# DavidSevic/gpu-nbody-simulation

Measured on AMD Instinct MI355X. Metric: body-steps/sec, higher is better.
Workload: dtype f32

## Files before the change

gpu-nbody-simulation_amd/csrc/bh_engine.hip:

```cpp
#include "../../include/bhgpu.h"

#include <hip/hip_runtime.h>

#include <algorithm>
#include <cmath>
#include <cstdio>
#include <cstdlib>
#include <cstring>
#include <string>
#include <type_traits>
#include <vector>

#include "bh_tree.hpp"
#include "bh_walk_exact.hpp"
#include "bh_walk_f64.hpp"
#include "bh_diag.hpp"
#include "bh_direct.hpp"
#include "bh_field.hpp"
#include "bh_init.hpp"
#include "bh_let.hpp"
#include "bh_migrate.hpp"
#include "bh_walk_fast.h"

using namespace bh;
// ... 18 lines not shown
};

}

struct bh_ctx {
    bh_config cfg{};
    int Dm = 0;
    enum class Mode { Exact, F64, Mixed, F32 };
    Mode mode = Mode::Exact;
    bool tree64() const { return mode == Mode::Exact || mode == Mode::F64; }
    bool state64() const { return mode != Mode::F32; }
    bool compat = true;
    bool exact_thresholds = false;
    int device = 0;
    hipStream_t stream = nullptr;
    bool own_stream = false;
    int64_t n = 0;
    bool uploaded = false, tree_valid = false;
    int64_t internal_cap = 0, node_cap = 0;
    int64_t bfs_max = 12288;
    int exact_bpw = 0;
    int walk_split = 0;
    bool walk_asm = true;
    int sort_bucket = 1;
    bool last_sort_bucket = false, last_sort_packed = false;
    int64_t samples_n = -1;
    uint64_t *splitters = nullptr;
    uint16_t *sort_dig = nullptr;
    int build_items = 0;
    bool hilbert = false;
    int partial_count = 0;
    double *bslots = nullptr;
    bool slots_valid = false;
    bool slots_dirty = true;

    void *pos = nullptr, *vel = nullptr, *mass = nullptr, *force = nullptr;
    void *pos2 = nullptr, *vel2 = nullptr, *mass2 = nullptr, *force2 = nullptr;
    uint32_t *orig = nullptr, *orig2 = nullptr;
    bool orig_identity = true;
    int reorder_every = 16;
    int64_t builds = 0;
    float2 *spos = nullptr;
    float4 *sstate = nullptr;
    float *smass = nullptr;
    uint64_t *keys[2] = {nullptr, nullptr};
    uint32_t *vals[2] = {nullptr, nullptr};
// ... 477 lines not shown
        }, c->compat);
        return BH_OK;
    });
}

int launch_walk_f32(bh_ctx *c, const WalkRange &w, const WalkChoice &k)
{
    WalkFastArgs a{};
    a.quads = c->qf; a.aux = c->aux; a.partial = w.partial; a.spos = c->spos; a.smass = c->smass; a.perm = c->perm;
    a.pos = (float2 *)c->pos; a.vel = (float2 *)c->vel;
    a.state64 = c->state64() ? 1 : 0;
    a.sstate = c->sstate;
    a.acc_out = (float2 *)c->force; a.ctr = c->ctr;
    a.lo = w.lo; a.hi = w.hi; a.G = (float)c->cfg.G; a.dt = (float)c->cfg.dt;
    a.integrate = w.integrate ? 1 : 0; a.to_sorted = w.to_sorted ? 1 : 0;
    a.n_trees = c->let_mode ? c->world : 0; a.self_rank = c->let_mode ? c->rank : -1;
    a.part = w.part; a.acc_part = c->acc_part;
    a.forest_base = c->forest_base; a.let_cap = c->let_cap;
    c->exp.walk_args(a);
    a.group_cost = (w.lo == 0 && w.hi == c->n) ? c->group_cost : nullptr;
    a.bucket_consts = c->walk_consts;
    a.slots = w.slots;
    a.body_counts = w.stats ? c->body_counts : nullptr;
    const bool lds = (c->cfg.flags & BH_FLAG_LDS_STACK) != 0;
    a.pair_limit = std::max(0, 116 - 3 * c->Dm);
    int split = (c->cfg.flags & BH_FLAG_WALK_NO_SPLIT) || c->cfg.n_threads > 0 ? 1 : c->walk_split;
    if (split <= 0) {
        const int64_t groups = (w.hi - w.lo + kWave - 1) / kWave;
        split = groups <= (c->let_mode ? 512 : 768) ? 8 : groups <= 3072 ? 4 : 1;
    }
    if (3 * c->Dm + 2 > kWave) split = 1;
    const int per_record = walk_fast_split_effective(a, lds, split) ? kWave : kBlock;
    if (w.partial) c->partial_count = (int)blocks_for(w.hi - w.lo, per_record);
    return each_pass(c, w, per_record, [&](int64_t plo, int64_t phi, unsigned) -> int {
        a.lo = plo; a.hi = phi; a.partial = w.partial ? w.partial + 4 * ((plo - w.lo) / per_record) : nullptr;
        BH_HIP(c, launch_walk_fast(a, lds, w.stats, split, k.use_asm, c->stream));
        return BH_OK;
    });
}

int enqueue_walk(bh_ctx *c, bool integrate, bool to_sorted, int part = 0)
{
    WalkRange w{};
    owned_range(c, &w.lo, &w.hi);
    if (w.hi <= w.lo) return BH_OK;
    w.integrate = integrate; w.to_sorted = to_sorted; w.part = part;
// ... 79 lines not shown
    if (cfg->max_depth < 1 || cfg->max_depth > 32)
        return fail(nullptr, BH_ERR_ARG, "bh_create: max_depth must be 1..32");
    if (!(cfg->theta > 0.0)) return fail(nullptr, BH_ERR_ARG, "bh_create: theta must be > 0");
    if (cfg->precision != BH_PRECISION_F64_EXACT && cfg->precision != BH_PRECISION_F32 &&
        cfg->precision != BH_PRECISION_MIXED && cfg->precision != BH_PRECISION_F64)
        return fail(nullptr, BH_ERR_ARG, "bh_create: unknown precision");
    int ndev = 0;
    if (hipGetDeviceCount(&ndev) != hipSuccess || ndev <= 0)
        return fail(nullptr, BH_ERR_NO_DEVICE, "bh_create: no HIP device (libbhgpu has no CPU fallback)");
    if (cfg->device < 0 || cfg->device >= ndev)
        return fail(nullptr, BH_ERR_ARG, "bh_create: device ordinal out of range");

    bh_ctx *c = new bh_ctx();
    c->cfg = *cfg;
    c->Dm = cfg->max_depth - 1;
    c->mode = cfg->precision == BH_PRECISION_F64_EXACT ? Mode::Exact
            : cfg->precision == BH_PRECISION_F64       ? Mode::F64
            : cfg->precision == BH_PRECISION_MIXED     ? Mode::Mixed : Mode::F32;
    c->compat = cfg->reference_compat != 0;
    c->device = cfg->device;
    if (const char *e = std::getenv("BH_WALK_SPLIT")) c->walk_split = std::atoi(e);
    if (const char *e = std::getenv("BH_EXACT_BPW")) { const int b = std::atoi(e); c->exact_bpw = (b >= 1 && b <= kWave && (b & (b - 1)) == 0) ? b : 0; }
    if (const char *e = std::getenv("BH_WALK_ASM")) c->walk_asm = std::atoi(e) != 0;
    if (const char *e = std::getenv("BH_EXACT_BFS_MAX")) c->bfs_max = std::max(0, std::atoi(e));
    c->exact_thresholds = c->mode == Mode::Exact && c->walk_asm && !(cfg->flags & BH_FLAG_WALK_PORTABLE);
    if (const char *e = std::getenv("BH_SORT_PACK")) c->sort_pack = std::atoi(e) != 0;
    if (const char *e = std::getenv("BH_SORT_BUCKET")) c->sort_bucket = std::atoi(e);
    if (const char *e = std::getenv("BH_BUILD_ITEMS")) c->build_items = std::atoi(e);
    if (const char *e = std::getenv("BH_REORDER_EVERY")) c->reorder_every = std::max(0, std::atoi(e));
    c->hilbert = !c->tree64();
    if (const char *e = std::getenv("BH_HILBERT")) c->hilbert = !c->tree64() && std::atoi(e) != 0;
    auto bail = [&](int rc) { g_create_error = c->err; bh_destroy(c); return rc; };

    if (hipSetDevice(c->device) != hipSuccess) { c->err = "hipSetDevice failed"; return bail(BH_ERR_DEVICE); }
    if (hipStreamCreateWithFlags(&c->stream, hipStreamNonBlocking) != hipSuccess) {
        c->err = "hipStreamCreate failed"; return bail(BH_ERR_DEVICE);
    }
    c->own_stream = true;

    const int64_t cap = std::max<int64_t>(cfg->capacity, 1);
    c->node_cap = cfg->node_capacity > 0 ? cfg->node_capacity : 8 * cap + 1024;
    if (c->Dm < 15) {
        int64_t full = 0, wdt = 1;
        for (int l = 0; l <= c->Dm; ++l) { full += wdt; wdt *= 4; }
        c->node_cap = std::min(c->node_cap, std::max<int64_t>(full, 1));
    }
    c->internal_cap = (c->node_cap - 1) / 4;

    const size_t rs = c->state64() ? sizeof(double) : sizeof(float);
    int rc = 0;
    auto A = [&](auto **pp, size_t count) { if (!rc) rc = dev_alloc(c, pp, count); };
    { char *t; A(&t, cap * 2 * rs); c->pos = t; }
    { char *t; A(&t, cap * 2 * rs); c->vel = t; }
    { char *t; A(&t, cap * rs); c->mass = t; }
    { char *t; A(&t, cap * 2 * (c->tree64() ? sizeof(double) : sizeof(float))); c->force = t; }
    if (!c->tree64()) {
        { char *t; A(&t, cap * 2 * rs); c->pos2 = t; }
        { char *t; A(&t, cap * 2 * rs); c->vel2 = t; }
        { char *t; A(&t, cap * rs); c->mass2 = t; }
        { char *t; A(&t, cap * 2 * sizeof(float)); c->force2 = t; }
        A(&c->orig, cap); A(&c->orig2, cap);
    }
    A(&c->keys[0], cap); A(&c->keys[1], cap); A(&c->vals[0], cap); A(&c->vals[1], cap);
    A(&c->cnt, cap + 1);
    { const size_t nbl = std::max<size_t>(blocks_for(cap, kSortTile), blocks_for(std::min<int64_t>(cap, 1 << 22), kBlock * kSmallItems));
      const size_t big = (cap > kBucketMaxN) ? (size_t)kBucketsBig * blocks_for(std::min<int64_t>(cap, kBucketMaxNBig), kBlock * kSmallItems) : 0;
      A(&c->radix_counts, std::max<size_t>((size_t)(1 << kSortBits) * nbl, big));
      A(&c->bsum_sort, 2 * kBucketStartOffset);
      A(&c->splitters, kBucketsBig);
      A(&c->sort_dig, (size_t)std::min<int64_t>(cap, kBucketMaxNBig) + 16);
    }
    const size_t scan_tiles = std::max<size_t>(blocks_for(cap + 1, kTile), blocks_for(std::min<int64_t>(cap, 1 << 22) + 1, kBlock * kSmallItems)) + 8;
    A(&c->bsum_u32, scan_tiles);
    A(&c->partial, 4 * (std::max<size_t>(1024, blocks_for(cap, kWave)) + 2));
    A(&c->box, 8); A(&c->bslots, 4 * kBoundSlots);
    A(&c->ctr, 1);
    if (c->tree64()) {
        { NodeD *g0 = nullptr; LinkD *l0 = nullptr; A(&g0, c->node_cap + 4); A(&l0, c->node_cap + 4);
          if (!rc) { c->gd = g0 + 3; c->ld = l0 + 3; } }
        A(&c->self_node, c->internal_cap + 1); A(&c->com_pending, c->internal_cap + 1); A(&c->cell_depth, c->internal_cap + 1);
        A(&c->cell_first, c->internal_cap + 1);
    } else {
        A(&c->qf, c->internal_cap + 1); A(&c->aux, 4 * (c->internal_cap + 1));
        A(&c->cell_first, c->internal_cap + 1);
        A(&c->gid, cap); A(&c->group_cost, cap / kWave + 2); A(&c->walk_consts, 4);
        A(&c->coarse, cap / 256 + 2);
        A(&c->spos, cap); A(&c->sstate, cap + 64 * kBlock + 1024); A(&c->smass, cap);
        A(&c->terms, cap + 1); A(&c->bsum_d3, scan_tiles);
    }
    if (rc) return bail(rc);
    if (hipMemset(c->ctr, 0, sizeof(TreeCounters)) != hipSuccess) { c->err = "hipMemset failed"; return bail(BH_ERR_DEVICE); }
    if (!c->tree64()) {
        const void *wc[4] = {c->aux, c->spos, c->smass, nullptr};
        if (hipMemcpy(c->walk_consts, wc, sizeof(wc), hipMemcpyHostToDevice) != hipSuccess) { c->err = "hipMemcpy failed"; return bail(BH_ERR_DEVICE); }
    }
    if (!c->tree64() && c->exp.create(cap) != hipSuccess) { c->err = "experiment hooks: allocation failed"; return bail(BH_ERR_DEVICE); }
    auto create = [](auto &evs) { for (auto &e : evs) if (hipEventCreate(&e) != hipSuccess) return false; return true; };
    if (!create(c->ev_step) || !create(c->ev_build) || !create(c->ev_grp) || !create(c->ev_let)) {
        c->err = "hipEventCreate failed"; return bail(BH_ERR_DEVICE);
    }
    *out = c;
    return BH_OK;
}

void bh_destroy(bh_ctx *c)
{
    if (!c) return;
    (void)hipSetDevice(c->device);
// ... 387 lines not shown
        const int64_t *tg = targets ? c->direct_targets : nullptr;
        if (c->state64())
            hipLaunchKernelGGL((direct_forces_kernel<double2, double>), dim3(blocks_for(k, kBlock)), dim3(kBlock), 0, c->stream,
                               (const double2 *)c->pos, (const double *)c->mass, slot_of, tg, t0, k, c->n, c->cfg.G, c->direct_out);
        else
            hipLaunchKernelGGL((direct_forces_kernel<float2, float>), dim3(blocks_for(k, kBlock)), dim3(kBlock), 0, c->stream,
                               (const float2 *)c->pos, (const float *)c->mass, slot_of, tg, t0, k, c->n, c->cfg.G, c->direct_out);
        BH_HIP(c, hipGetLastError());
        BH_HIP(c, hipMemcpyAsync(out + 2 * t0, c->direct_out, k * sizeof(double2), hipMemcpyDeviceToHost, c->stream));
        BH_HIP(c, hipStreamSynchronize(c->stream));
    }
    return BH_OK;
}

static int check_walk(bh_ctx *c, double *out)
{
    const size_t cap = (size_t)std::max<int64_t>(c->cfg.capacity, 1);
    int rc = BH_OK;
    if (!c->check_force) {
        char *f = nullptr;
        rc = dev_alloc(c, &f, cap * 2 * (c->tree64() ? sizeof(double) : sizeof(float)));
        c->check_force = f;
        if (!rc && !c->ctr_save) rc = dev_alloc(c, &c->ctr_save, 1);
        if (!rc && c->group_cost) rc = dev_alloc(c, &c->check_cost, cap / kWave + 2);
        if (rc) return rc;
    }
    if ((c->cfg.flags & BH_FLAG_WALK_STATS) && !c->check_counts) { if ((rc = dev_alloc(c, &c->check_counts, cap))) return rc; }
    const int64_t launches = c->walk_launches;
    const bool cost_valid = c->group_cost_valid;
    constexpr size_t wc_off = offsetof(TreeCounters, visits), wc_bytes = sizeof(TreeCounters) - wc_off;
    BH_HIP(c, hipMemcpyAsync((char *)c->ctr_save + wc_off, (char *)c->ctr + wc_off, wc_bytes, hipMemcpyDeviceToDevice, c->stream));
    rc = enqueue_quiet_build(c);
    if (!rc) {
        auto swap_outputs = [&] {
            std::swap(c->force, c->check_force);
            std::swap(c->body_counts, c->check_counts);
            std::swap(c->group_cost, c->check_cost);
        };
        swap_outputs();
        rc = enqueue_walk(c, false, false);
        swap_outputs();
    }
    c->walk_launches = launches;
    c->group_cost_valid = cost_valid;
    BH_HIP(c, hipMemcpyAsync((char *)c->ctr + wc_off, (char *)c->ctr_save + wc_off, wc_bytes, hipMemcpyDeviceToDevice, c->stream));
    if (!rc) rc = check_overflow(c);
    return rc ? rc : forces_or_accels(c, c->check_force, out, true);
// ... 731 lines not shown
```

gpu-nbody-simulation_amd/csrc/bh_walk_fast.h:

```cpp
#pragma once

#include <hip/hip_runtime.h>
#include <stdint.h>

namespace bh {

struct QuadF;
struct NodeAux;
struct TreeCounters;

struct WalkFastArgs {
    const QuadF *quads;
    const NodeAux *aux;
    const float2 *spos;
    const float *smass;
    const uint32_t *perm;
    float2 *pos, *vel;
    int32_t state64;
    float4 *sstate;
    float2 *acc_out;
    TreeCounters *ctr;
    double *partial;
    int64_t lo, hi;
    float G, dt;
    int integrate, to_sorted;
    uint32_t nblocks, pad0;
    const void *bucket_consts;
    uint32_t *group_cost;
    int32_t pair_limit;
    uint64_t *timeline;
    int32_t n_trees, self_rank;
    int32_t part;
    float2 *acc_part;
    int64_t forest_base, let_cap;
    double *slots;
    uint32_t *body_counts;
};

hipError_t launch_walk_fast(const WalkFastArgs &a, bool lds_stack, bool stats, int split, bool use_asm, hipStream_t st);
inline bool walk_fast_split_effective(const WalkFastArgs &a, bool lds_stack, int split)
{
    return split > 1 && !lds_stack && a.n_trees <= 56;
}

}
```

gpu-nbody-simulation_amd/csrc/bh_walk_fast.hip:

```cpp
#include "bh_prims.hpp"
#include "bh_nodes.hpp"
#include "bh_bounds.hpp"
#include "bh_walk_fast.h"
#include <cstdlib>

namespace bh {

#define BH_CONSTANT __attribute__((address_space(4)))

extern "C" __device__ int bh_writelane_i32(int value, int lane, int old) __asm("llvm.amdgcn.writelane.i32");

template <typename T>
__device__ __forceinline__ const T BH_CONSTANT *as_constant(const T *p)
{
#pragma clang diagnostic push
#pragma clang diagnostic ignored "-Wold-style-cast"
    return (const T BH_CONSTANT *)p;
#pragma clang diagnostic pop
}

typedef int32_t v16i __attribute__((ext_vector_type(16)));
typedef int32_t v4i __attribute__((ext_vector_type(4)));
typedef int32_t v2i __attribute__((ext_vector_type(2)));
struct QuadRegs { v16i g; v4i c; };

__device__ __forceinline__ QuadRegs load_quad(const QuadF BH_CONSTANT *q)
{
    QuadRegs r;
#pragma clang diagnostic push
#pragma clang diagnostic ignored "-Wold-style-cast"
    r.g = *(const v16i BH_CONSTANT *)q;
    r.c = *(const v4i BH_CONSTANT *)((const char BH_CONSTANT *)q + 64);
#pragma clang diagnostic pop
    return r;
}

#if defined(BH_ASM_GUARD) && BH_ASM_GUARD
#define BH_LOOP_GUARD "s_cmp_gt_u32 %[cost], 0x100000\n s_cbranch_scc1 Ldone_%=\n"
#else
#define BH_LOOP_GUARD ""
#endif
#define BH_FORCE_MATH(MS, MASK)                                                                     \
    "v_mul_f32_e32 v26, " MS ", v25\n"                                                              \
    "v_mul_f32_e32 v26, v25, v26\n"                                                                 \
    "v_mul_f32_e32 v24, v25, v26\n"                                                                 \
    "v_fmac_f32_e32 v28, v24, v22\n"                                                                \
    "v_fmac_f32_e32 v29, v24, v23\n"                                                                \
    "s_mov_b64 exec, " MASK "\n"
#define BH_CHILD_HEAD(XY, MS, TS, MASK, SPAIR, TAG)                                                 \
    "s_cmp_eq_u32 " MS ", 0\n"                                                                      \
    "s_cbranch_scc1 Lnext" TAG "_%=\n"                                                              \
    "v_pk_add_f32 v[22:23], " XY ", v[20:21] neg_lo:[0,1] neg_hi:[0,1]\n"                           \
    "s_nop 0\n"                                                                                     \
    "v_mul_f32_e32 v24, v23, v23\n"                                                                 \
    "v_fmac_f32_e32 v24, v22, v22\n"                                                                \
    "v_cmpx_lt_f32_e32 vcc, " TS ", v24\n"                                                          \
    "v_rsq_f32_e32 v25, v24\n"                                                                      \
    "s_andn2_b64 " SPAIR ", " MASK ", vcc\n"                                                        \
    "s_cbranch_scc0 Lforce" TAG "_%=\n"
#define BH_CHILD_T(XY, MS, TS, CS, MASK, SPAIR, SLO, SHI, TAG, PUSHCHK)                             \
    BH_CHILD_HEAD(XY, MS, TS, MASK, SPAIR, TAG)                                                     \
    "s_cmp_eq_u32 " CS ", -1\n"                                                                     \
    "s_cbranch_scc1 Lforce" TAG "_%=\n"                                                             \
// ... 27 lines not shown
    BH_FORCE_MATH(MS, MASK)                                                                         \
    "s_branch " NEXT "_%=\n"
#define BH_PUSHCHK(TAG) "s_bitcmp1_b32 m0, 6\n s_cbranch_scc1 LpushHi" TAG "_%=\n"
#define BH_NOCHK(TAG) ""
#define BH_PUSH_HI(CS, SLO, SHI, TAG)                                                               \
    "LpushHi" TAG "_%=:\n"                                                                          \
    "v_writelane_b32 v33, " CS ", m0\n"                                                             \
    "v_writelane_b32 v34, " SLO ", m0\n"                                                            \
    "v_writelane_b32 v35, " SHI ", m0\n"                                                            \
    "s_branch LpushBack" TAG "_%=\n"
#define BH_POP_FAST(IDX, LO, HI)                                                                    \
    "s_lshl_b64 exec, 1, m0\n"                                                                      \
    "v_readfirstlane_b32 " IDX ", v30\n v_readfirstlane_b32 " LO ", v31\n v_readfirstlane_b32 " HI ", v32\n"
#define BH_POP(IDX, LO, HI, TAG)                                                                    \
    "s_lshl_b64 exec, 1, m0\n"                                                                      \
    "s_bitcmp1_b32 m0, 6\n"                                                                         \
    "s_cbranch_scc1 LpopHi" TAG "_%=\n"                                                             \
    "v_readfirstlane_b32 " IDX ", v30\n v_readfirstlane_b32 " LO ", v31\n v_readfirstlane_b32 " HI ", v32\n" \
    "LpopBack" TAG "_%=:\n"
#define BH_POP_HI(IDX, LO, HI, TAG)                                                                 \
    "LpopHi" TAG "_%=:\n"                                                                           \
    "v_readfirstlane_b32 " IDX ", v33\n v_readfirstlane_b32 " LO ", v34\n v_readfirstlane_b32 " HI ", v35\n" \
    "s_branch LpopBack" TAG "_%=\n"
#define BH_ITERATION(SFX, POPA, POPB, CHK)                                                              \
                   \
    "s_cmp_gt_i32 s72, -1\n"                                                                        \
    "s_cbranch_scc1 LAn" SFX "_%=\n"                                                                \
    "s_sub_u32 m0, m0, 1\n"                                  \
    "s_cbranch_scc1 LAe" SFX "_%=\n"                                                                \
    POPA                                                                                            \
    "s_cmp_lt_i32 s68, 0\n"                                                                         \
    "s_cbranch_scc1 Lspecial_%=\n"                                                                  \
    "s_branch LAr" SFX "_%=\n"                                                                      \
    "LAe" SFX "_%=:\n"                                                                              \
    "s_mov_b32 m0, 0\n"                                                                             \
    "s_cmp_lt_i32 s70, 0\n"                                                                         \
    "s_cbranch_scc1 Ldone_%=\n"                                                                     \
    "s_mov_b32 s68, s70\n"                                                                          \
    "s_mov_b64 s[44:45], s[46:47]\n"                                                                \
    "s_mov_b32 s70, -1\n"                                                                           \
    "s_branch LAr" SFX "_%=\n"                                                                      \
    "LAn" SFX "_%=:\n"                                                                              \
    "s_mov_b32 s68, s72\n"                                   \
    "LAr" SFX "_%=:\n"                                    \
    "s_mul_i32 s69, s68, 0x50\n"                                                                    \
    "s_load_dwordx16 s[24:39], %[quads], s69\n"                                                     \
    "s_load_dwordx4 s[40:43], %[quads], s69 offset:0x40\n"                                          \
        \
    "s_cmp_gt_i32 s70, -1\n"                                                                        \
    "s_cbranch_scc1 LBn" SFX "_%=\n"                                                                \
    "s_mov_b64 s[46:47], 0\n"                                             \
    "s_cmp_eq_u32 m0, 0\n"                                                                          \
    "s_cbranch_scc1 LW" SFX "_%=\n"                                                                 \
    "s_cmp_gt_u32 m0, %[plim]\n"                                                                    \
    "s_cbranch_scc1 LW" SFX "_%=\n"                                                                 \
    "s_sub_u32 m0, m0, 1\n"                                                                         \
    POPB                                                                                            \
    "s_cmp_lt_i32 s70, 0\n"                                                                         \
    "s_cbranch_scc1 Lunpop" SFX "_%=\n"                                                             \
    "LBn" SFX "_%=:\n"                                                                              \
    "s_mul_i32 s71, s70, 0x50\n"                                                                    \
    "s_load_dwordx16 s[48:63], %[quads], s71\n"                                                     \
    "s_load_dwordx4 s[64:67], %[quads], s71 offset:0x40\n"                                          \
    "LW" SFX "_%=:\n"                                                                               \
    "s_mov_b64 exec, s[44:45]\n"                                                                    \
    "s_waitcnt lgkmcnt(0)\n"                                                                                    \
    "s_setprio 0\n"                                                                                 \
                                                         \
    BH_CHILD_F("s[24:25]", "s32", "s36", "s40", "s[44:45]", SFX "A0f", CHK(SFX "A0f"))              \
    BH_CHILD_F("s[26:27]", "s33", "s37", "s41", "s[44:45]", SFX "A1f", CHK(SFX "A1f"))              \
    BH_CHILD_F("s[28:29]", "s34", "s38", "s42", "s[44:45]", SFX "A2f", CHK(SFX "A2f"))              \
    BH_CHILD_F("s[30:31]", "s35", "s39", "s43", "s[44:45]", SFX "A3f", CHK(SFX "A3f"))              \
    "s_mov_b32 s72, -1\n"                                                  \
    "s_branch LphB" SFX "_%=\n"                                                                     \
      \
    "LA1t" SFX "_%=:\n"                                                                             \
    BH_CHILD_T("s[26:27]", "s33", "s37", "s41", "s[44:45]", "s[70:71]", "s70", "s71", SFX "A1t", CHK(SFX "A1t")) \
    "LA2t" SFX "_%=:\n"                                                                             \
    BH_CHILD_T("s[28:29]", "s34", "s38", "s42", "s[44:45]", "s[70:71]", "s70", "s71", SFX "A2t", CHK(SFX "A2t")) \
    "LA3t" SFX "_%=:\n"                                                                             \
    BH_CHILD_T("s[30:31]", "s35", "s39", "s43", "s[44:45]", "s[70:71]", "s70", "s71", SFX "A3t", CHK(SFX "A3t")) \
    "LAet" SFX "_%=:\n"                                                                             \
    "s_mov_b64 s[44:45], s[68:69]\n"                      \
    "s_mov_b32 s70, -1\n"                                 \
    "LphB" SFX "_%=:\n"                                                                             \
    "s_cmp_eq_u64 s[46:47], 0\n"                                                                    \
    "s_cbranch_scc1 Lloop_%=\n"                                           \
    "s_mov_b64 exec, s[46:47]\n"                                                                    \
    "s_cmp_gt_u32 m0, %[plim]\n"                          \
    "s_cbranch_scc1 LBover" SFX "_%=\n"                                                             \
    BH_CHILD_F("s[48:49]", "s56", "s60", "s64", "s[46:47]", SFX "B0f", CHK(SFX "B0f"))              \
    BH_CHILD_F("s[50:51]", "s57", "s61", "s65", "s[46:47]", SFX "B1f", CHK(SFX "B1f"))              \
    BH_CHILD_F("s[52:53]", "s58", "s62", "s66", "s[46:47]", SFX "B2f", CHK(SFX "B2f"))              \
    BH_CHILD_F("s[54:55]", "s59", "s63", "s67", "s[46:47]", SFX "B3f", CHK(SFX "B3f"))              \
    "s_mov_b32 s70, -1\n"                                                                           \
    "s_branch Lloop_%=\n"                                                                           \
    "LB0t" SFX "_%=:\n"                                                                             \
    BH_CHILD_T("s[48:49]", "s56", "s60", "s64", "s[46:47]", "s[24:25]", "s24", "s25", SFX "B0t", CHK(SFX "B0t")) \
    "LB1t" SFX "_%=:\n"                                                                             \
    BH_CHILD_T("s[50:51]", "s57", "s61", "s65", "s[46:47]", "s[24:25]", "s24", "s25", SFX "B1t", CHK(SFX "B1t")) \
    "LB2t" SFX "_%=:\n"                                                                             \
    BH_CHILD_T("s[52:53]", "s58", "s62", "s66", "s[46:47]", "s[24:25]", "s24", "s25", SFX "B2t", CHK(SFX "B2t")) \
    "LB3t" SFX "_%=:\n"                                                                             \
    BH_CHILD_T("s[54:55]", "s59", "s63", "s67", "s[46:47]", "s[24:25]", "s24", "s25", SFX "B3t", CHK(SFX "B3t")) \
    "LBet" SFX "_%=:\n"                                                                             \
    "s_mov_b64 s[46:47], s[68:69]\n"                      \
    "s_branch Lloop_%=\n"                                                                           \
    "Lunpop" SFX "_%=:\n"                                 \
    "s_add_u32 m0, m0, 1\n"                                                                         \
    "s_mov_b32 s70, -1\n"                                                                           \
    "s_mov_b64 s[46:47], 0\n"                                                                       \
    "s_branch LW" SFX "_%=\n"                                                                       \
    "LBover" SFX "_%=:\n"                                   \
    "s_mov_b32 s70, -1\n"                                                                           \
    "s_branch LB0t" SFX "_%=\n"                                                                     \
    BH_TAKE("s32", "s40", "s[44:45]", "s72", SFX "A0f", "LA1t" SFX)                                 \
    BH_TAKE("s33", "s41", "s[44:45]", "s72", SFX "A1f", "LA2t" SFX)                                 \
    BH_TAKE("s34", "s42", "s[44:45]", "s72", SFX "A2f", "LA3t" SFX)                                 \
    BH_TAKE("s35", "s43", "s[44:45]", "s72", SFX "A3f", "LAet" SFX)                                 \
    BH_TAKE("s56", "s64", "s[46:47]", "s70", SFX "B0f", "LB1t" SFX)                                 \
    BH_TAKE("s57", "s65", "s[46:47]", "s70", SFX "B1f", "LB2t" SFX)                                 \
    BH_TAKE("s58", "s66", "s[46:47]", "s70", SFX "B2f", "LB3t" SFX)                                 \
    BH_TAKE("s59", "s67", "s[46:47]", "s70", SFX "B3f", "LBet" SFX)
#define BH_HI_STUBS(SFX)                                                                            \
    BH_PUSH_HI("s40", "s68", "s69", SFX "A0f") BH_PUSH_HI("s41", "s68", "s69", SFX "A1f")          \
    BH_PUSH_HI("s42", "s68", "s69", SFX "A2f") BH_PUSH_HI("s43", "s68", "s69", SFX "A3f")          \
    BH_PUSH_HI("s41", "s70", "s71", SFX "A1t") BH_PUSH_HI("s42", "s70", "s71", SFX "A2t")          \
    BH_PUSH_HI("s43", "s70", "s71", SFX "A3t")                                                     \
    BH_PUSH_HI("s64", "s68", "s69", SFX "B0f") BH_PUSH_HI("s65", "s68", "s69", SFX "B1f")          \
    BH_PUSH_HI("s66", "s68", "s69", SFX "B2f") BH_PUSH_HI("s67", "s68", "s69", SFX "B3f")          \
    BH_PUSH_HI("s64", "s24", "s25", SFX "B0t") BH_PUSH_HI("s65", "s24", "s25", SFX "B1t")          \
    BH_PUSH_HI("s66", "s24", "s25", SFX "B2t") BH_PUSH_HI("s67", "s24", "s25", SFX "B3t")

#define BH_TREE_LOOP(LIMITCHK) \
     \
    "Lloop_%=:\n" \
    "s_add_u32 %[cost], %[cost], 1\n" \
    BH_LOOP_GUARD LIMITCHK \
    "s_setprio 2\n" \
    "s_cmp_gt_u32 m0, 56\n" \
    "s_cbranch_scc1 LloopChk_%=\n" \
    BH_ITERATION("F", BH_POP_FAST("s68", "s44", "s45"), BH_POP_FAST("s70", "s46", "s47"), BH_NOCHK) \
    "LloopChk_%=:\n"  \
    BH_ITERATION("C", BH_POP("s68", "s44", "s45", "A"), BH_POP("s70", "s46", "s47", "B"), BH_PUSHCHK) \
    BH_HI_STUBS("C") \
    BH_POP_HI("s68", "s44", "s45", "A") \
    BH_POP_HI("s70", "s46", "s47", "B") \
     \
     \
     \
    "Lspecial_%=:\n" \
    "s_cmp_eq_u32 s68, -1\n" \
    "s_cbranch_scc1 Lloop_%=\n" \
    "s_load_dwordx8 s[56:63], %[consts], 0x0\n"  \
    "s_sub_i32 s68, -2, s68\n" \
    "s_lshl_b32 s69, s68, 3\n" \
    "s_mov_b64 exec, s[44:45]\n" \
    "s_waitcnt lgkmcnt(0)\n" \
    "s_load_dwordx2 s[48:49], s[56:57], s69\n"  \
    "s_waitcnt lgkmcnt(0)\n" \
    "s_cmp_lt_i32 s49, 1\n" \
    "s_cbranch_scc1 Lloop_%=\n" \
    "s_add_u32 s49, s48, s49\n" \
    "Lbody_%=:\n" \
    "s_lshl_b32 s69, s48, 3\n" \
    "s_load_dwordx2 s[50:51], s[58:59], s69\n" \
    "s_lshl_b32 s69, s48, 2\n" \
    "s_load_dword s52, s[60:61], s69\n" \
    "s_add_u32 s48, s48, 1\n" \
    "s_waitcnt lgkmcnt(0)\n" \
    "v_pk_add_f32 v[22:23], s[50:51], v[20:21] neg_lo:[0,1] neg_hi:[0,1]\n" \
    "s_cmp_lt_u32 s48, s49\n"  \
    "v_mul_f32_e32 v24, v23, v23\n" \
    "v_fmac_f32_e32 v24, v22, v22\n" \
    "v_cmpx_lt_f32_e32 vcc, 0, v24\n" \
    "v_rsq_f32_e32 v25, v24\n" \
    "s_nop 0\n"  \
    "v_mul_f32_e32 v26, s52, v25\n" \
    "v_mul_f32_e32 v26, v25, v26\n" \
    "v_mul_f32_e32 v24, v25, v26\n" \
    "v_fmac_f32_e32 v28, v24, v22\n" \
    "v_fmac_f32_e32 v29, v24, v23\n" \
    "s_mov_b64 exec, s[44:45]\n" \
    "s_cbranch_scc1 Lbody_%=\n" \
    "s_branch Lloop_%=\n"

__device__ __forceinline__ uint32_t walk_tree_asm(const QuadF BH_CONSTANT *quads, const void BH_CONSTANT *consts,
                                                   int32_t root, uint64_t everyone, int32_t pair_limit, float px,
                                                   float py, float &ax, float &ay)
{
    uint32_t cost;
    asm volatile(
        "v_mov_b32_e32 v20, %[px]\n"
        "v_mov_b32_e32 v21, %[py]\n"
        "v_mov_b32_e32 v28, %[ax]\n"
        "v_mov_b32_e32 v29, %[ay]\n"
        "s_mov_b32 m0, 0\n"
        "s_mov_b32 s70, -1\n"
        "s_mov_b32 s72, -1\n"
        "s_mov_b32 %[cost], 1\n"
        "s_branch LArF_%=\n"
        BH_TREE_LOOP("")
        "Ldone_%=:\n"
        "s_setprio 0\n"
        "s_mov_b64 exec, -1\n"
        "v_mov_b32_e32 %[ax], v28\n"
        "v_mov_b32_e32 %[ay], v29\n"
        : [ax] "+v"(ax), [ay] "+v"(ay), [cost] "=&s"(cost), "+{s68}"(root), "+{s[44:45]}"(everyone)
        : [quads] "s"(quads), [consts] "s"(consts), [px] "v"(px), [py] "v"(py), [plim] "s"(pair_limit)
        : "s24", "s25", "s26", "s27", "s28", "s29", "s30", "s31", "s32", "s33", "s34", "s35", "s36", "s37", "s38", "s39",
          "s40", "s41", "s42", "s43", "s46", "s47", "s48", "s49", "s50", "s51", "s52", "s53", "s54", "s55",
          "s56", "s57", "s58", "s59", "s60", "s61", "s62", "s63", "s64", "s65", "s66", "s67", "s69", "s70", "s71", "s72",
          "m0", "vcc", "scc", "memory",
          "v20", "v21", "v22", "v23", "v24", "v25", "v26", "v27", "v28", "v29", "v30", "v31", "v32", "v33", "v34", "v35");
    return cost;
}
__device__ __forceinline__ int32_t walk_list_asm(const QuadF BH_CONSTANT *quads, const void BH_CONSTANT *consts,
                                                 int32_t in_base, int32_t in_lo, int32_t in_hi, int32_t mine,
                                                 float px, float py, float &ax, float &ay, int32_t &out_base,
                                                 int32_t &out_lo, int32_t &out_hi)
{
    int32_t sp;
    asm volatile(
        "v_mov_b32_e32 v20, %[px]\n"
        "v_mov_b32_e32 v21, %[py]\n"
        "v_mov_b32_e32 v28, %[ax]\n"
        "v_mov_b32_e32 v29, %[ay]\n"
        "v_mov_b32_e32 v33, %[ib]\n"
        "v_mov_b32_e32 v34, %[il]\n"
        "v_mov_b32_e32 v35, %[ih]\n"
        "s_mov_b32 m0, 0\n"
        "s_mov_b32 s72, 0\n"
// ... 92 lines not shown
constexpr int kLdsStackDepth = 128;
constexpr int kSplitFrontier = 512;
constexpr int kSplitRound = 16;

template <bool LDS_STACK, bool STATS, int SPLIT, bool ASM = false>
__global__ __launch_bounds__(SPLIT > 1 ? kWave * SPLIT : kBlock) void walk_fast_kernel(WalkFastArgs a)
{
    static_assert(SPLIT == 1 || !LDS_STACK, "the split walk uses the register-lane stack");
    static_assert(!ASM || (!LDS_STACK && !STATS), "the assembly loops serve the default configuration");
    __shared__ int32_t s_base[LDS_STACK ? kWavesPerBlock : 1][LDS_STACK ? kLdsStackDepth : 1];
    __shared__ uint64_t s_mask[LDS_STACK ? kWavesPerBlock : 1][LDS_STACK ? kLdsStackDepth : 1];
    constexpr int FCAP = SPLIT > 1 ? kSplitFrontier : 1;
    __shared__ int32_t fr_base[2][FCAP], fr_lo[2][FCAP], fr_hi[2][FCAP];
    __shared__ int32_t f_cnt[SPLIT > 1 ? SPLIT : 1];
    __shared__ float2 f_red[SPLIT > 1 ? SPLIT : 1][SPLIT > 1 ? kWave : 1];

    if (a.ctr->overflow) return;
#ifdef BHGPU_EXPERIMENTS
    const uint64_t dbg_t0 = a.timeline ? __builtin_amdgcn_s_memrealtime() : 0;
    const uint64_t dbg_c0 = a.timeline ? __builtin_amdgcn_s_memtime() : 0;
#endif
    const uint32_t lb = blockIdx.x;
    if (lb >= a.nblocks) return;
    const int lane = lane_id(), w = wave_id();
    const int64_t s = SPLIT > 1 ? a.lo + (int64_t)lb * kWave + lane : a.lo + (int64_t)lb * kBlock + threadIdx.x;
    bool valid = s < a.hi;
    const float2 p = valid ? a.spos[s] : float2{0.f, 0.f};
    asm volatile("" ::"v"(p.x), "v"(p.y));
    float ax = 0.f, ay = 0.f;
    if (a.part == 2 && valid && (SPLIT == 1 || w == 0)) { const float2 t = a.acc_part[s]; ax = t.x; ay = t.y; }
    asm volatile("" : "+v"(ax), "+v"(ay));
    unsigned long long n_vis = 0, n_int = 0, n_wave = 0, n_quad = 0;
    uint32_t my_int = 0;
    uint32_t cost = 0;

    const QuadF BH_CONSTANT *quads = as_constant(a.quads);
    const NodeAux BH_CONSTANT *aux = as_constant(a.aux);
    const float2 BH_CONSTANT *cpos = as_constant(a.spos);
    const float BH_CONSTANT *cmass = as_constant(a.smass);

    int32_t v_base = 0, v_lo = 0, v_hi = 0;
    int32_t v_base2 = 0, v_lo2 = 0, v_hi2 = 0;
    int sp = 0;

    bool h_free = false;
    int32_t h_idx = -1;
// ... 176 lines not shown
                        if (base <= -2) { bucket(-base - 2, mask); continue; }
                        if (base < 0) continue;
                        do {
                            const QuadRegs q = load_quad(quads + base);
                            eval_quad(q, mask);
                        } while (pop_quad(base, mask));
                    }
                }
                __syncthreads();
            }
            cur ^= 1;
            F = produced;
        }
        f_red[w][lane] = float2{ax, ay};
        __syncthreads();
        if (w == 0) {
#pragma unroll
            for (int k = 1; k < SPLIT; ++k) { ax += f_red[k][lane].x; ay += f_red[k][lane].y; }
        }
        valid = valid && (w == 0);
    } else {
        const uint64_t everyone = __ballot(valid);
        const int32_t t_first = (a.part == 2) ? 0 : -1, t_end = (a.part == 1) ? 0 : a.n_trees;
        for (int32_t t = t_first; t < t_end; ++t) {
            if (t >= 0 && t == a.self_rank) continue;
            int32_t base = (t < 0) ? 0 : (int32_t)(a.forest_base + (int64_t)t * a.let_cap);
            if (ASM) {
                cost += walk_tree_asm(quads, as_constant(a.bucket_consts), base, everyone, a.pair_limit, p.x, p.y, ax, ay);
                continue;
            }
            {
                int32_t na = -1, nb = -1;
                uint64_t nam = 0, nbm = 0;
                bool first = true;
                for (;;) {
                    int32_t bA, bB = -1;
                    uint64_t mA, mB = 0;
                    ++cost;
                    if (first) { bA = base; mA = everyone; first = false; }
                    else {
                        if (na >= 0) { bA = na; mA = nam; }
                        else if (sp > 0) {
                            pop_raw(bA, mA);
                            if (bA < 0) {
                                if (bA <= -2) bucket(-bA - 2, mA);
                                continue;
                            }
                        } else if (nb >= 0) { bA = nb; mA = nbm; nb = -1; }
                        else break;
                        if (nb >= 0) { bB = nb; mB = nbm; }
                        else if (sp > 0 && sp <= a.pair_limit) {
// ... 56 lines not shown
                e.vel[body] = v;
                e.pos[body] = np;
            }
        }
    }
    const double bx = e.state64 ? np64.x : (double)np.x, by = e.state64 ? np64.y : (double)np.y;
    if (SPLIT > 1) {
        if ((e.slots || e.partial) && w == 0) {
            const double xlo = wave_min(valid ? bx : (double)INFINITY), xhi = wave_max(valid ? bx : -(double)INFINITY);
            const double ylo = wave_min(valid ? by : (double)INFINITY), yhi = wave_max(valid ? by : -(double)INFINITY);
            if (lane == 0) {
                if (e.partial) {
                    double *o = e.partial + 4 * (size_t)lb;
                    o[0] = xlo; o[1] = xhi; o[2] = ylo; o[3] = yhi;
                }
                if (e.slots) bounds_to_slot(xlo, xhi, ylo, yhi, e.slots, (uint32_t)lb);
            }
        }
    } else if (e.slots || e.partial) block_bounds(valid, bx, by, e.slots, e.partial ? e.partial + 4 * (size_t)lb : nullptr);
#ifdef BHGPU_EXPERIMENTS
    if (e.timeline && lane == 0) {
        const int64_t wv = (int64_t)blockIdx.x * (blockDim.x >> 6) + w;
        const uint64_t c1 = __builtin_amdgcn_s_memtime(), t1 = __builtin_amdgcn_s_memrealtime();
        e.timeline[6 * wv + 0] = dbg_t0;
        e.timeline[6 * wv + 1] = t1;
        e.timeline[6 * wv + 2] = (uint64_t)__builtin_amdgcn_s_getreg((4 << 0) | (0 << 6) | (31 << 11));
        e.timeline[6 * wv + 3] = cost;
        e.timeline[6 * wv + 4] = dbg_c0;
        e.timeline[6 * wv + 5] = c1;
    }
#endif
    if (e.group_cost && lane == 0 && (SPLIT == 1 || w == 0)) {
        const int64_t g = (SPLIT > 1 ? e.lo + (int64_t)lb * kWave : e.lo + (int64_t)lb * kBlock + (int64_t)w * kWave) >> 6;
        if (e.part == 2) e.group_cost[g] += cost;
        else e.group_cost[g] = cost;
    }
    if (STATS && e.body_counts && s < e.hi && my_int) atomicAdd(&e.body_counts[e.perm[s]], my_int);
    if (STATS && lane == 0) {
        atomicAdd(&e.ctr->visits, n_vis);
        atomicAdd(&e.ctr->interactions, n_int);
        atomicAdd(&e.ctr->wave_nodes, n_wave);
        atomicAdd(&e.ctr->wave_quads, n_quad);
    }
}

template <bool L, bool S, int SPLIT = 1, bool ASM = false>
static hipError_t launch(WalkFastArgs a, hipStream_t st)
{
    const int64_t cnt = a.hi - a.lo;
    if (cnt <= 0) return hipSuccess;
    constexpr int per_group = SPLIT > 1 ? kWave : kBlock;
    a.nblocks = (uint32_t)((cnt + per_group - 1) / per_group);
    hipLaunchKernelGGL((walk_fast_kernel<L, S, SPLIT, ASM>), dim3(a.nblocks), dim3(SPLIT > 1 ? kWave * SPLIT : kBlock), 0, st, a);
    return hipGetLastError();
}

template <bool S, bool ASM = false>
static hipError_t launch_split(const WalkFastArgs &a, int split, hipStream_t st)
{
    switch (split) {
    case 2: return launch<false, S, 2, ASM>(a, st);
    case 4: return launch<false, S, 4, ASM>(a, st);
    default: return launch<false, S, 8, ASM>(a, st);
    }
}

hipError_t launch_walk_fast(const WalkFastArgs &a, bool lds_stack, bool stats, int split, bool use_asm, hipStream_t st)
{
    if (use_asm && !lds_stack && !stats && !walk_fast_split_effective(a, lds_stack, split))
        return launch<false, false, 1, true>(a, st);
    if (walk_fast_split_effective(a, lds_stack, split))
        return stats ? launch_split<true>(a, split, st)
                     : (use_asm ? launch_split<false, true>(a, split, st) : launch_split<false>(a, split, st));
    if (lds_stack) return stats ? launch<true, true>(a, st) : launch<true, false>(a, st);
    return stats ? launch<false, true>(a, st) : launch<false, false>(a, st);
}

}
```

Before: 2.370 billion.

## Add cost-based wave priority scheduling to the last round of the asm tree walk

In the last resident round of the inline-asm Barnes-Hut walk, each wave now uses the previous step's per-group cost to pick its hardware priority (s_setprio). A wave starts at high priority and drops through tiers as it passes quartiles of its expected cost, so the most expensive waves in the tail get scheduled first. The aim is to shorten the load-imbalance tail at the end of the kernel. This adds an occupancy query at context creation, new kernel arguments, and a duplicated asm loop body with extra branches, which raises code size and the risk of instruction-cache or register pressure.

Result: faster. 2.489 billion (median of 6 runs) (+5.0%).

```diff
diff --git a/gpu-nbody-simulation_amd/csrc/bh_engine.hip b/gpu-nbody-simulation_amd/csrc/bh_engine.hip
--- a/gpu-nbody-simulation_amd/csrc/bh_engine.hip
+++ b/gpu-nbody-simulation_amd/csrc/bh_engine.hip
@@ -64,6 +64,9 @@
     int exact_bpw = 0;
     int walk_split = 0;
     bool walk_asm = true;
+    int walk_prio = 1;
+    uint32_t resident_blocks = 0;
+    uint32_t walk_prio_rounds = 10;
     int sort_bucket = 1;
     bool last_sort_bucket = false, last_sort_packed = false;
     int64_t samples_n = -1;
@@ -587,6 +590,10 @@
     a.bucket_consts = c->walk_consts;
     a.slots = w.slots;
     a.body_counts = w.stats ? c->body_counts : nullptr;
+    const bool few_rounds = blocks_for(w.hi - w.lo, kBlock) <= (uint64_t)c->walk_prio_rounds * c->resident_blocks;
+    a.prio = (a.group_cost && w.part == 0 && a.n_trees == 0 && w.pass == w.hi - w.lo && few_rounds) ? c->walk_prio : 0;
+    a.prev_valid = (a.prio != 0 && c->group_cost_valid) ? 1 : 0;
+    a.resident_blocks = c->resident_blocks;
     const bool lds = (c->cfg.flags & BH_FLAG_LDS_STACK) != 0;
     a.pair_limit = std::max(0, 116 - 3 * c->Dm);
     int split = (c->cfg.flags & BH_FLAG_WALK_NO_SPLIT) || c->cfg.n_threads > 0 ? 1 : c->walk_split;
@@ -712,6 +719,14 @@
     if (const char *e = std::getenv("BH_WALK_SPLIT")) c->walk_split = std::atoi(e);
     if (const char *e = std::getenv("BH_EXACT_BPW")) { const int b = std::atoi(e); c->exact_bpw = (b >= 1 && b <= kWave && (b & (b - 1)) == 0) ? b : 0; }
     if (const char *e = std::getenv("BH_WALK_ASM")) c->walk_asm = std::atoi(e) != 0;
+    if (const char *e = std::getenv("BH_WALK_PRIO")) {
+        const int v = std::atoi(e);
+#ifdef BHGPU_EXPERIMENTS
+        c->walk_prio = (v >= 0 && v <= 3) ? v : 1;
+#else
+        c->walk_prio = v != 0 ? 1 : 0;
+#endif
+    }
     if (const char *e = std::getenv("BH_EXACT_BFS_MAX")) c->bfs_max = std::max(0, std::atoi(e));
     c->exact_thresholds = c->mode == Mode::Exact && c->walk_asm && !(cfg->flags & BH_FLAG_WALK_PORTABLE);
     if (const char *e = std::getenv("BH_SORT_PACK")) c->sort_pack = std::atoi(e) != 0;
@@ -727,6 +742,15 @@
         c->err = "hipStreamCreate failed"; return bail(BH_ERR_DEVICE);
     }
     c->own_stream = true;
+    if (!c->tree64()) {
+        int per_cu = 0, cus = 0;
+        if (walk_fast_blocks_per_cu(&per_cu) != hipSuccess || hipDeviceGetAttribute(&cus, hipDeviceAttributeMultiprocessorCount, c->device) != hipSuccess) {
+            c->err = "walk occupancy query failed"; return bail(BH_ERR_DEVICE);
+        }
+        c->resident_blocks = (uint32_t)(std::min(std::max(per_cu, 1), 8) * std::max(cus, 1));
+        if (const char *e = std::getenv("BH_WALK_PRIO_ROUNDS")) c->walk_prio_rounds = (uint32_t)std::min(std::max(std::atoi(e), 0), 1 << 20);
+        if (const char *e = std::getenv("BH_WALK_RESIDENT_BLOCKS")) { const long long v = std::atoll(e); if (v >= 1) c->resident_blocks = (uint32_t)std::min<long long>(v, 0x7fffffffLL); }
+    }
 
     const int64_t cap = std::max<int64_t>(cfg->capacity, 1);
     c->node_cap = cfg->node_capacity > 0 ? cfg->node_capacity : 8 * cap + 1024;
@@ -773,7 +797,7 @@
     } else {
         A(&c->qf, c->internal_cap + 1); A(&c->aux, 4 * (c->internal_cap + 1));
         A(&c->cell_first, c->internal_cap + 1);
-        A(&c->gid, cap); A(&c->group_cost, cap / kWave + 2); A(&c->walk_consts, 4);
+        A(&c->gid, cap); A(&c->group_cost, cap / kWave + 8); A(&c->walk_consts, 4);
         A(&c->coarse, cap / 256 + 2);
         A(&c->spos, cap); A(&c->sstate, cap + 64 * kBlock + 1024); A(&c->smass, cap);
         A(&c->terms, cap + 1); A(&c->bsum_d3, scan_tiles);
@@ -1207,7 +1231,7 @@
         rc = dev_alloc(c, &f, cap * 2 * (c->tree64() ? sizeof(double) : sizeof(float)));
         c->check_force = f;
         if (!rc && !c->ctr_save) rc = dev_alloc(c, &c->ctr_save, 1);
-        if (!rc && c->group_cost) rc = dev_alloc(c, &c->check_cost, cap / kWave + 2);
+        if (!rc && c->group_cost) rc = dev_alloc(c, &c->check_cost, cap / kWave + 8);
         if (rc) return rc;
     }
     if ((c->cfg.flags & BH_FLAG_WALK_STATS) && !c->check_counts) { if ((rc = dev_alloc(c, &c->check_counts, cap))) return rc; }
diff --git a/gpu-nbody-simulation_amd/csrc/bh_walk_fast.h b/gpu-nbody-simulation_amd/csrc/bh_walk_fast.h
--- a/gpu-nbody-simulation_amd/csrc/bh_walk_fast.h
+++ b/gpu-nbody-simulation_amd/csrc/bh_walk_fast.h
@@ -35,9 +35,12 @@
     int64_t forest_base, let_cap;
     double *slots;
     uint32_t *body_counts;
+    int32_t prio, prev_valid;
+    uint32_t resident_blocks, pad1;
 };
 
 hipError_t launch_walk_fast(const WalkFastArgs &a, bool lds_stack, bool stats, int split, bool use_asm, hipStream_t st);
+hipError_t walk_fast_blocks_per_cu(int *blocks);
 inline bool walk_fast_split_effective(const WalkFastArgs &a, bool lds_stack, int split)
 {
     return split > 1 && !lds_stack && a.n_trees <= 56;
diff --git a/gpu-nbody-simulation_amd/csrc/bh_walk_fast.hip b/gpu-nbody-simulation_amd/csrc/bh_walk_fast.hip
--- a/gpu-nbody-simulation_amd/csrc/bh_walk_fast.hip
+++ b/gpu-nbody-simulation_amd/csrc/bh_walk_fast.hip
@@ -36,9 +36,25 @@
 }
 
 #if defined(BH_ASM_GUARD) && BH_ASM_GUARD
-#define BH_LOOP_GUARD "s_cmp_gt_u32 %[cost], 0x100000\n s_cbranch_scc1 Ldone_%=\n"
+#define BH_LOOP_GUARD_U "s_cmp_gt_u32 %[cost], 0x100000\n s_cbranch_scc1 Ldone_%=\n"
+#define BH_LOOP_GUARD_I "s_cmp_gt_i32 %[cost], 0x100000\n s_cbranch_scc1 Ldone_%=\n"
 #else
-#define BH_LOOP_GUARD ""
+#define BH_LOOP_GUARD_U ""
+#define BH_LOOP_GUARD_I ""
+#endif
+#define BH_STEP_FLIP "s_add_u32 %[cost], %[cost], 1\n" BH_LOOP_GUARD_U
+#define BH_STEP_PROGRESS "s_add_u32 %[cost], %[cost], 1\n s_cbranch_scc1 Lretier_%=\n LloopR_%=:\n" BH_LOOP_GUARD_I
+#ifdef BHGPU_EXPERIMENTS
+#define BH_STEP_HIGH "s_add_u32 %[cost], %[cost], 1\n s_cbranch_scc1 LloopRl_%=\n" BH_LOOP_GUARD_I
+#define BH_STEP_LOW "s_add_u32 %[cost], %[cost], 1\n LloopRl_%=:\n" BH_LOOP_GUARD_I
+#define BH_TWO_CLASS_ENTRY "s_cmp_eq_u32 s69, 2\n s_cbranch_scc1 LenterH_%=\n"
+#define BH_TWO_CLASS_LOOPS \
+    "LenterH_%=:\n s_setprio 3\n v_readlane_b32 s69, v27, 0\n s_sub_u32 %[cost], 1, s69\n s_branch LArFh_%=\n" \
+    BH_TREE_LOOP("", "h", BH_STEP_HIGH, "s_setprio 3\n", "s_setprio 2\n") \
+    BH_TREE_LOOP("", "l", BH_STEP_LOW, "s_setprio 1\n", "s_setprio 0\n")
+#else
+#define BH_TWO_CLASS_ENTRY ""
+#define BH_TWO_CLASS_LOOPS ""
 #endif
 #define BH_FORCE_MATH(MS, MASK)                                                                     \
     "v_mul_f32_e32 v26, " MS ", v25\n"                                                              \
@@ -112,7 +128,7 @@
     "LpopHi" TAG "_%=:\n"                                                                           \
     "v_readfirstlane_b32 " IDX ", v33\n v_readfirstlane_b32 " LO ", v34\n v_readfirstlane_b32 " HI ", v35\n" \
     "s_branch LpopBack" TAG "_%=\n"
-#define BH_ITERATION(SFX, POPA, POPB, CHK)                                                              \
+#define BH_ITERATION(SFX, POPA, POPB, CHK, LP, PWAITED)                                                          \
                    \
     "s_cmp_gt_i32 s72, -1\n"                                                                        \
     "s_cbranch_scc1 LAn" SFX "_%=\n"                                                                \
@@ -120,7 +136,7 @@
     "s_cbranch_scc1 LAe" SFX "_%=\n"                                                                \
     POPA                                                                                            \
     "s_cmp_lt_i32 s68, 0\n"                                                                         \
-    "s_cbranch_scc1 Lspecial_%=\n"                                                                  \
+    "s_cbranch_scc1 Lspecial" LP "_%=\n"                                                                  \
     "s_branch LAr" SFX "_%=\n"                                                                      \
     "LAe" SFX "_%=:\n"                                                                              \
     "s_mov_b32 m0, 0\n"                                                                             \
@@ -155,7 +171,7 @@
     "LW" SFX "_%=:\n"                                                                               \
     "s_mov_b64 exec, s[44:45]\n"                                                                    \
     "s_waitcnt lgkmcnt(0)\n"                                                                                    \
-    "s_setprio 0\n"                                                                                 \
+    PWAITED                                                                                         \
                                                          \
     BH_CHILD_F("s[24:25]", "s32", "s36", "s40", "s[44:45]", SFX "A0f", CHK(SFX "A0f"))              \
     BH_CHILD_F("s[26:27]", "s33", "s37", "s41", "s[44:45]", SFX "A1f", CHK(SFX "A1f"))              \
@@ -175,7 +191,7 @@
     "s_mov_b32 s70, -1\n"                                 \
     "LphB" SFX "_%=:\n"                                                                             \
     "s_cmp_eq_u64 s[46:47], 0\n"                                                                    \
-    "s_cbranch_scc1 Lloop_%=\n"                                           \
+    "s_cbranch_scc1 Lloop" LP "_%=\n"                                           \
     "s_mov_b64 exec, s[46:47]\n"                                                                    \
     "s_cmp_gt_u32 m0, %[plim]\n"                          \
     "s_cbranch_scc1 LBover" SFX "_%=\n"                                                             \
@@ -184,7 +200,7 @@
     BH_CHILD_F("s[52:53]", "s58", "s62", "s66", "s[46:47]", SFX "B2f", CHK(SFX "B2f"))              \
     BH_CHILD_F("s[54:55]", "s59", "s63", "s67", "s[46:47]", SFX "B3f", CHK(SFX "B3f"))              \
     "s_mov_b32 s70, -1\n"                                                                           \
-    "s_branch Lloop_%=\n"                                                                           \
+    "s_branch Lloop" LP "_%=\n"                                                                           \
     "LB0t" SFX "_%=:\n"                                                                             \
     BH_CHILD_T("s[48:49]", "s56", "s60", "s64", "s[46:47]", "s[24:25]", "s24", "s25", SFX "B0t", CHK(SFX "B0t")) \
     "LB1t" SFX "_%=:\n"                                                                             \
@@ -195,7 +211,7 @@
     BH_CHILD_T("s[54:55]", "s59", "s63", "s67", "s[46:47]", "s[24:25]", "s24", "s25", SFX "B3t", CHK(SFX "B3t")) \
     "LBet" SFX "_%=:\n"                                                                             \
     "s_mov_b64 s[46:47], s[68:69]\n"                      \
-    "s_branch Lloop_%=\n"                                                                           \
+    "s_branch Lloop" LP "_%=\n"                                                                           \
     "Lunpop" SFX "_%=:\n"                                 \
     "s_add_u32 m0, m0, 1\n"                                                                         \
     "s_mov_b32 s70, -1\n"                                                                           \
@@ -222,26 +238,25 @@
     BH_PUSH_HI("s64", "s24", "s25", SFX "B0t") BH_PUSH_HI("s65", "s24", "s25", SFX "B1t")          \
     BH_PUSH_HI("s66", "s24", "s25", SFX "B2t") BH_PUSH_HI("s67", "s24", "s25", SFX "B3t")
 
-#define BH_TREE_LOOP(LIMITCHK) \
+#define BH_TREE_LOOP(LIMITCHK, LP, STEP, PSTART, PWAITED) \
      \
-    "Lloop_%=:\n" \
-    "s_add_u32 %[cost], %[cost], 1\n" \
-    BH_LOOP_GUARD LIMITCHK \
-    "s_setprio 2\n" \
+    "Lloop" LP "_%=:\n" \
+    STEP LIMITCHK \
+    PSTART \
     "s_cmp_gt_u32 m0, 56\n" \
-    "s_cbranch_scc1 LloopChk_%=\n" \
-    BH_ITERATION("F", BH_POP_FAST("s68", "s44", "s45"), BH_POP_FAST("s70", "s46", "s47"), BH_NOCHK) \
-    "LloopChk_%=:\n"  \
-    BH_ITERATION("C", BH_POP("s68", "s44", "s45", "A"), BH_POP("s70", "s46", "s47", "B"), BH_PUSHCHK) \
-    BH_HI_STUBS("C") \
-    BH_POP_HI("s68", "s44", "s45", "A") \
-    BH_POP_HI("s70", "s46", "s47", "B") \
+    "s_cbranch_scc1 LloopChk" LP "_%=\n" \
+    BH_ITERATION("F" LP, BH_POP_FAST("s68", "s44", "s45"), BH_POP_FAST("s70", "s46", "s47"), BH_NOCHK, LP, PWAITED) \
+    "LloopChk" LP "_%=:\n"  \
+    BH_ITERATION("C" LP, BH_POP("s68", "s44", "s45", "A" LP), BH_POP("s70", "s46", "s47", "B" LP), BH_PUSHCHK, LP, PWAITED) \
+    BH_HI_STUBS("C" LP) \
+    BH_POP_HI("s68", "s44", "s45", "A" LP) \
+    BH_POP_HI("s70", "s46", "s47", "B" LP) \
      \
      \
      \
-    "Lspecial_%=:\n" \
+    "Lspecial" LP "_%=:\n" \
     "s_cmp_eq_u32 s68, -1\n" \
-    "s_cbranch_scc1 Lloop_%=\n" \
+    "s_cbranch_scc1 Lloop" LP "_%=\n" \
     "s_load_dwordx8 s[56:63], %[consts], 0x0\n"  \
     "s_sub_i32 s68, -2, s68\n" \
     "s_lshl_b32 s69, s68, 3\n" \
@@ -250,9 +265,9 @@
     "s_load_dwordx2 s[48:49], s[56:57], s69\n"  \
     "s_waitcnt lgkmcnt(0)\n" \
     "s_cmp_lt_i32 s49, 1\n" \
-    "s_cbranch_scc1 Lloop_%=\n" \
+    "s_cbranch_scc1 Lloop" LP "_%=\n" \
     "s_add_u32 s49, s48, s49\n" \
-    "Lbody_%=:\n" \
+    "Lbody" LP "_%=:\n" \
     "s_lshl_b32 s69, s48, 3\n" \
     "s_load_dwordx2 s[50:51], s[58:59], s69\n" \
     "s_lshl_b32 s69, s48, 2\n" \
@@ -272,12 +287,12 @@
     "v_fmac_f32_e32 v28, v24, v22\n" \
     "v_fmac_f32_e32 v29, v24, v23\n" \
     "s_mov_b64 exec, s[44:45]\n" \
-    "s_cbranch_scc1 Lbody_%=\n" \
-    "s_branch Lloop_%=\n"
+    "s_cbranch_scc1 Lbody" LP "_%=\n" \
+    "s_branch Lloop" LP "_%=\n"
 
 __device__ __forceinline__ uint32_t walk_tree_asm(const QuadF BH_CONSTANT *quads, const void BH_CONSTANT *consts,
-                                                   int32_t root, uint64_t everyone, int32_t pair_limit, float px,
-                                                   float py, float &ax, float &ay)
+                                                   int32_t root, uint64_t everyone, int32_t pair_limit, int32_t sched,
+                                                   float px, float py, float &ax, float &ay)
 {
     uint32_t cost;
     asm volatile(
@@ -285,19 +300,55 @@
         "v_mov_b32_e32 v21, %[py]\n"
         "v_mov_b32_e32 v28, %[ax]\n"
         "v_mov_b32_e32 v29, %[ay]\n"
+        "v_mov_b32_e32 v27, %[sched]\n"
         "s_mov_b32 m0, 0\n"
         "s_mov_b32 s70, -1\n"
         "s_mov_b32 s72, -1\n"
         "s_mov_b32 %[cost], 1\n"
-        "s_branch LArF_%=\n"
-        BH_TREE_LOOP("")
+        "v_readlane_b32 s69, v27, 10\n"
+        "s_cmp_eq_u32 s69, 0\n"
+        "s_cbranch_scc1 LArF_%=\n"
+        BH_TWO_CLASS_ENTRY
+        "s_setprio 3\n"
+        "v_readlane_b32 s69, v27, 0\n"
+        "s_sub_u32 %[cost], 1, s69\n"
+        "s_branch LArFp_%=\n"
+        BH_TREE_LOOP("", "", BH_STEP_FLIP, "s_setprio 2\n", "s_setprio 0\n")
+        BH_TREE_LOOP("", "p", BH_STEP_PROGRESS, "", "")
+        BH_TWO_CLASS_LOOPS
+        "Lretier_%=:\n"
+        "v_readlane_b32 s24, v27, 8\n"
+        "s_cmp_lg_u32 s24, 0\n"
+        "s_cbranch_scc1 Lretier1_%=\n"
+        "s_setprio 2\n"
+        "s_branch LretierSet_%=\n"
+        "Lretier1_%=:\n"
+        "s_cmp_lg_u32 s24, 1\n"
+        "s_cbranch_scc1 Lretier2_%=\n"
+        "s_setprio 1\n"
+        "s_branch LretierSet_%=\n"
+        "Lretier2_%=:\n"
+        "s_setprio 0\n"
+        "LretierSet_%=:\n"
+        "s_add_u32 s24, s24, 1\n"
+        "s_min_u32 s24, s24, 3\n"
+        "v_writelane_b32 v27, s24, 8\n"
+        "v_readlane_b32 s25, v27, s24\n"
+        "s_sub_u32 %[cost], %[cost], s25\n"
+        "v_readlane_b32 s24, v27, 9\n"
+        "s_add_u32 s24, s24, s25\n"
+        "s_nop 0\n"
+        "v_writelane_b32 v27, s24, 9\n"
+        "s_branch LloopR_%=\n"
         "Ldone_%=:\n"
         "s_setprio 0\n"
+        "v_readlane_b32 s24, v27, 9\n"
         "s_mov_b64 exec, -1\n"
+        "s_add_u32 %[cost], %[cost], s24\n"
         "v_mov_b32_e32 %[ax], v28\n"
         "v_mov_b32_e32 %[ay], v29\n"
         : [ax] "+v"(ax), [ay] "+v"(ay), [cost] "=&s"(cost), "+{s68}"(root), "+{s[44:45]}"(everyone)
-        : [quads] "s"(quads), [consts] "s"(consts), [px] "v"(px), [py] "v"(py), [plim] "s"(pair_limit)
+        : [quads] "s"(quads), [consts] "s"(consts), [px] "v"(px), [py] "v"(py), [plim] "s"(pair_limit), [sched] "v"(sched)
         : "s24", "s25", "s26", "s27", "s28", "s29", "s30", "s31", "s32", "s33", "s34", "s35", "s36", "s37", "s38", "s39",
           "s40", "s41", "s42", "s43", "s46", "s47", "s48", "s49", "s50", "s51", "s52", "s53", "s54", "s55",
           "s56", "s57", "s58", "s59", "s60", "s61", "s62", "s63", "s64", "s65", "s66", "s67", "s69", "s70", "s71", "s72",
@@ -436,6 +487,15 @@
 #endif
     const uint32_t lb = blockIdx.x;
     if (lb >= a.nblocks) return;
+    const WalkFastArgs BH_CONSTANT *kp;
+    {
+#pragma clang diagnostic push
+#pragma clang diagnostic ignored "-Wold-style-cast"
+        kp = (const WalkFastArgs BH_CONSTANT *)__builtin_amdgcn_kernarg_segment_ptr();
+#pragma clang diagnostic pop
+    }
+    asm volatile("" : "+s"(kp));
+    const int32_t prio = ASM ? kp->prio : 0;
     const int lane = lane_id(), w = wave_id();
     const int64_t s = SPLIT > 1 ? a.lo + (int64_t)lb * kWave + lane : a.lo + (int64_t)lb * kBlock + threadIdx.x;
     bool valid = s < a.hi;
@@ -658,11 +718,36 @@
     } else {
         const uint64_t everyone = __ballot(valid);
         const int32_t t_first = (a.part == 2) ? 0 : -1, t_end = (a.part == 1) ? 0 : a.n_trees;
+        int32_t sched = 0;
+        if (ASM) {
+            if (prio != 0) {
+                sched = lane == 10 ? 1 : 0;
+#ifdef BHGPU_EXPERIMENTS
+                if (prio == 2) sched = lane == 10 ? 2 : 0;
+#endif
+                bool last_round = kp->nblocks - lb <= kp->resident_blocks;
+#ifdef BHGPU_EXPERIMENTS
+                if (prio == 3) last_round = true;
+#endif
+                if (last_round && everyone != 0 && kp->prev_valid) {
+                    const int64_t g = (kp->lo + (int64_t)lb * kBlock + (int64_t)w * kWave) >> 6;
+                    const uint32_t prev = as_constant(kp->group_cost)[__builtin_amdgcn_readfirstlane((int32_t)g)];
+                    if (prev >= 16) {
+                        uint32_t q1 = prev >> 2;
+                        const uint32_t q2 = prev >> 1, q3 = (3 * prev) >> 2;
+#ifdef BHGPU_EXPERIMENTS
+                        if (prio == 2) q1 = q2;
+#endif
+                        sched = (lane == 0 || lane == 9) ? (int32_t)q1 : lane == 1 ? (int32_t)(q2 - q1) : lane == 2 ? (int32_t)(q3 - q2) : sched;
+                    }
+                }
+            }
+        }
         for (int32_t t = t_first; t < t_end; ++t) {
             if (t >= 0 && t == a.self_rank) continue;
             int32_t base = (t < 0) ? 0 : (int32_t)(a.forest_base + (int64_t)t * a.let_cap);
             if (ASM) {
-                cost += walk_tree_asm(quads, as_constant(a.bucket_consts), base, everyone, a.pair_limit, p.x, p.y, ax, ay);
+                cost += walk_tree_asm(quads, as_constant(a.bucket_consts), base, everyone, a.pair_limit, sched, p.x, p.y, ax, ay);
                 continue;
             }
             {
@@ -765,12 +850,13 @@
     if (e.timeline && lane == 0) {
         const int64_t wv = (int64_t)blockIdx.x * (blockDim.x >> 6) + w;
         const uint64_t c1 = __builtin_amdgcn_s_memtime(), t1 = __builtin_amdgcn_s_memrealtime();
-        e.timeline[6 * wv + 0] = dbg_t0;
-        e.timeline[6 * wv + 1] = t1;
-        e.timeline[6 * wv + 2] = (uint64_t)__builtin_amdgcn_s_getreg((4 << 0) | (0 << 6) | (31 << 11));
-        e.timeline[6 * wv + 3] = cost;
-        e.timeline[6 * wv + 4] = dbg_c0;
-        e.timeline[6 * wv + 5] = c1;
+        e.timeline[7 * wv + 0] = dbg_t0;
+        e.timeline[7 * wv + 1] = t1;
+        e.timeline[7 * wv + 2] = (uint64_t)__builtin_amdgcn_s_getreg((4 << 0) | (0 << 6) | (31 << 11));
+        e.timeline[7 * wv + 3] = cost;
+        e.timeline[7 * wv + 4] = dbg_c0;
+        e.timeline[7 * wv + 5] = c1;
+        e.timeline[7 * wv + 6] = (uint64_t)__builtin_amdgcn_s_getreg((20 << 0) | (0 << 6) | (3 << 11));
     }
 #endif
     if (e.group_cost && lane == 0 && (SPLIT == 1 || w == 0)) {
@@ -808,6 +894,11 @@
     }
 }
 
+hipError_t walk_fast_blocks_per_cu(int *blocks)
+{
+    return hipOccupancyMaxActiveBlocksPerMultiprocessor(blocks, walk_fast_kernel<false, false, 1, true>, kBlock, 0);
+}
+
 hipError_t launch_walk_fast(const WalkFastArgs &a, bool lds_stack, bool stats, int split, bool use_asm, hipStream_t st)
 {
     if (use_asm && !lds_stack && !stats && !walk_fast_split_effective(a, lds_stack, split))
```
